# dropbox/lepton

Hardware: AMD Instinct MI355X
Metric: encode+decode MB/s (JPEG bytes/sec), bit-exact round trip (higher is better)
Workload: dtype int16/u8 (integer coder, no floating point)

## Files before the change

### lepton_amd/csrc/lep_dec4.h

```cpp
#pragma once
#include "lep_v3.h"
#include "lep_enc3.h"

namespace lep4 {
using namespace lep3;

#if LEP_ON_GPU && defined(LEP_MARKS)
#define LEP_MARK(name) __asm__ volatile("; MARK " name)
#elif LEP_ON_GPU && defined(LEP_PROF)
#define LEP_MARK(name) prof_stamp(lep4::prof_slot(name))
#else
#define LEP_MARK(name) ((void)0)
#endif
#if LEP_ON_GPU && (defined(LEP_DEC4_PAD_VALU) || defined(LEP_DEC4_PAD_SALU) || defined(LEP_DEC4_PAD_LDS))
#define LEP_PAD8(x) x x x x x x x x
WDEV void pad_block(uint32_t seed, const void* lds) {
    (void)seed; (void)lds;
#ifdef LEP_DEC4_PAD_VALU
    { uint32_t o; for (int i = 0; i < LEP_DEC4_PAD_VALU / 8; ++i) __asm__ volatile(LEP_PAD8("v_add_u32 %0, %1, %1\n") : "=v"(o) : "v"(seed)); }
#endif
#ifdef LEP_DEC4_PAD_SALU
    { uint32_t o; const uint32_t u = uni(seed); for (int i = 0; i < LEP_DEC4_PAD_SALU / 8; ++i) __asm__ volatile(LEP_PAD8("s_add_u32 %0, %1, %1\n") : "=s"(o) : "s"(u) : "scc"); }
#endif
#ifdef LEP_DEC4_PAD_LDS
    { uint32_t o; const uint32_t a = (uint32_t)(uintptr_t)lds; for (int i = 0; i < LEP_DEC4_PAD_LDS / 8; ++i) __asm__ volatile(LEP_PAD8("ds_read_b32 %0, %1\n") "s_waitcnt lgkmcnt(0)\n" : "=v"(o) : "v"(a)); }
#endif
}
#else
WDEV void pad_block(uint32_t, const void*) {}
#endif
constexpr int prof_slot(const char* n) {
    const char* names[18] = {"staging", "prologue", "nz_prefetch", "nz_serial", "nz_update", "77_prefetch", "77_serial", "77_update", "lakhani",
                             "edge_prefetch", "edge_serial", "edge_update", "idct_dcpred", "dc_prefetch", "dc_serial", "dc_update", "publish", "store"};
    for (int i = 0; i < 18; ++i) {
        int k = 0;
        while (names[i][k] && names[i][k] == n[k]) ++k;
        if (!names[i][k] && !n[k]) return i;
    }
    return 31;
}

#ifndef LEP_DEC4_ROW_MAJOR
constexpr uint32_t kGS = 10 * 4;
WDEV uint32_t ctx4_exp7(int ci, int nb, int zz, int bsr) { return lep3::kExp7 + (((((uint32_t)ci * 49 + zz) * 12 + bsr) * 3) * 10 + nb) * 4; }
WDEV uint32_t ctx4_expx(int ci, int ne, int zig15, int bsr) { return lep3::kExpX + (((((uint32_t)ci * 15 + zig15) * 12 + bsr) * 3) * 10 + ne) * 4; }
WDEV uint32_t ctx4_res(int ci, int coord, int nb) { return lep3::kRes + ((((uint32_t)ci * 64 + coord) * 3) * 10 + nb) * 4; }
#else
constexpr uint32_t kGS = 4;
WDEV uint32_t ctx4_exp7(int ci, int nb, int zz, int bsr) { return lep3::ctx_exp7(ci, nb, zz, bsr); }
WDEV uint32_t ctx4_expx(int ci, int ne, int zig15, int bsr) { return lep3::ctx_expx(ci, ne, zig15, bsr); }
WDEV uint32_t ctx4_res(int ci, int coord, int nb) { return lep3::ctx_res(ci, coord, nb); }
#endif
WDEV uint32_t row_word(uint32_t base, int i) { return base + (uint32_t)(i >> 2) * kGS + (uint32_t)(i & 3); }

struct Dec4Shared {
    uint32_t sign[kSignWords];
    uint32_t resdc[kResDcWords];
    alignas(16) int32_t t[64];
    int32_t icos_x[64], icos_y[64];
    int32_t eprior[16];
    int16_t here[64], left[64], above[64], aleft[64];
    alignas(16) int16_t pix[64];
    uint16_t q[64];
    uint8_t thr[64], r2a[64], a2r[64], nzbin[64], bsr[64];
    uint8_t cj[32], cn[32];
    NSum ns_left, ns_above, ns_here;
    uint32_t inv24[512];
};
static_assert(sizeof(Dec4Shared) <= 160 * 1024 / 32, "Dec4Shared no longer fits 32 times into a CU's LDS");

WDEV int nzbin_of(int left) {
    return left < 16 ? (int)((0x7776666555443210ull >> (4 * left)) & 15) : (left < 21 ? 7 : (left < 32 ? 8 : 9));
}
WDEV int nzhi_of(int b) { return (int)((0xc5f50c2050c2040ull >> (6 * b)) & 63); }
#ifndef LEP_DEC4_CANDS
#define LEP_DEC4_CANDS 4
#endif
WDEV int combo_base(int j) { return (int)((0x1b65648d1c0ull >> (6 * j)) & 63); }

WDEV uint32_t inv24_of(uint32_t d) {
    if (d < 2) return 0;
    return (0x1000000u + d - 1) / d - ((d == 337 || d == 469) ? 1u : 0u);
}
WDEV uint32_t mul24(uint32_t a, uint32_t b) {
#if LEP_ON_GPU
    return __umul24(a, b);
#else
    return (uint32_t)(((uint64_t)(a & 0xffffff) * (b & 0xffffff)) & 0xffffffffu);
#endif
}
WDEV uint32_t mul24_low(uint32_t a, uint32_t b) {
#if LEP_ON_GPU
    uint32_t r;
    __asm__("v_mul_u32_u24 %0, %1, %2" : "=v"(r) : "v"(a), "v"(b));
    return r;
#else
    return mul24(a, b);
#endif
}
struct DivBy {
    uint32_t mul, shift;
    WDEV static uint32_t shift_of(uint32_t d) { return 31u - (uint32_t)__builtin_clz(d - 1); }
    WDEV static DivBy of(uint32_t d) {
        DivBy r;
        uint32_t s = 1;
        while (s < 31 && (1u << s) < d) ++s;
        uint32_t q = 0, rem = 1u << (s - 1);
        for (int i = 0; i < 32; ++i) {
            rem <<= 1; q <<= 1;
            if (rem >= d) { rem -= d; q |= 1u; }
        }
        r.mul = q + (rem ? 1u : 0u);
        r.shift = s - 1;
        return r;
    }
};
WDEV uint32_t mulhi_u32(uint32_t a, uint32_t b) {
#if LEP_ON_GPU
    return __umulhi(a, b);
#else
    return (uint32_t)(((uint64_t)a * b) >> 32);
#endif
}
WDEV int32_t div_by(int32_t n, uint32_t mul, uint32_t shift) {
    const int32_t sign = n >> 31;
    const uint32_t u = ((uint32_t)n ^ (uint32_t)sign) - (uint32_t)sign;
    const uint32_t q = mulhi_u32(u, mul) >> shift;
    return (int32_t)((q ^ (uint32_t)sign) - (uint32_t)sign);
}
WDEV uint32_t bupd_t(uint32_t w, uint32_t obs, const uint32_t* inv24) {
    const uint32_t f = (w & 255) + (obs ^ 1), t = ((w >> 8) & 255) + obs;
    uint32_t nw = f | (t << 8) | ((mul24(f << 8, inv24[f + t]) >> 24) << 16);
    if ((f | t) > 255) {
        const uint32_t f0 = w & 255, t0 = (w >> 8) & 255;
        if ((obs ? f0 : t0) == 1) nw = (w & 0xffff) | ((obs ? 0u : 255u) << 16);
        else {
            const uint32_t f2 = obs ? (1 + f0) >> 1 : 129u, t2 = obs ? 129u : (1 + t0) >> 1;
            nw = f2 | (t2 << 8) | ((mul24(f2 << 8, inv24[f2 + t2]) >> 24) << 16);
        }
    }
    return nw;
}
WDEV uint32_t bupd_u(uint32_t w, uint32_t obs, const uint32_t* inv24) {
    const uint32_t w2 = w + 1u + obs * 255u;
    const uint32_t f = w2 & 255u, t = (w2 >> 8) & 255u;
    if (ucond((f < t ? f : t) == 0)) {
        const uint32_t f0 = w & 255, t0 = (w >> 8) & 255;
        if (ucond((obs ? f0 : t0) == 1)) return (w & 0xffff) | ((obs ? 0u : 255u) << 16);
        const uint32_t f2 = obs ? (1 + f0) >> 1 : 129u, t2 = obs ? 129u : (1 + t0) >> 1;
        return f2 | (t2 << 8) | ((mul24(f2 << 8, inv24[f2 + t2]) >> 24) << 16);
    }
    return (w2 & 0xffffu) | (mul24_low(f, inv24[f + t]) & 0xff0000u);
}

WDEV uint64_t pair64(uint32_t hi, uint32_t lo) {
#if LEP_ON_GPU && !defined(LEP_DEC4_PAIR_OR)
    typedef uint32_t u32x2 __attribute__((ext_vector_type(2)));
    const u32x2 p = {lo, hi};
    return __builtin_bit_cast(uint64_t, p);
#else
    return ((uint64_t)hi << 32) | lo;
#endif
}
struct BoolDec4 {
    uint32_t vhi, vlo;
    int count;
    uint32_t range;
    const uint32_t* words;
    uint32_t first, end;
    uint32_t wi;
    uint32_t raw;

    WDEV uint32_t fetch(uint32_t k) const { return k * 4 < end ? words[k] : 0u; }
    WDEV void refill() {
        const uint32_t lo = wi * 4;
        uint32_t w = __builtin_bswap32(raw);
        int nbits = 32;
        if (lo + 4 > end) w = lo < end ? (w & ~(0xffffffffu >> ((end - lo) * 8))) : 0u;
        if (lo < first) { w <<= (first - lo) * 8; nbits -= (int)(first - lo) * 8; }
        const uint64_t add = ((uint64_t)w << 32) >> (count + 8);
        vhi |= (uint32_t)(add >> 32); vlo |= (uint32_t)add;
        count += nbits;
        ++wi;
        raw = fetch(wi);
    }
    WDEV void init_stream(const uint8_t* p, uint32_t n) {
        const uint32_t mis = (uint32_t)((uintptr_t)p & 3);
        words = reinterpret_cast<const uint32_t*>(p - mis);
        first = mis; end = mis + n;
        vhi = vec(0); vlo = vec(0); count = (int)vec((uint32_t)-8); range = vec(255); wi = 0;
        raw = fetch(0);
        refill();
        get(128);
    }
    WDEV uint32_t get(uint32_t prob) {
#if LEP_ON_GPU
        const uint32_t split = 1 + (__umul24(range - 1, prob) >> 8);
#else
        const uint32_t split = 1 + (((range - 1) * prob) >> 8);
#endif
        if (ucond(count < 0)) refill();
        const uint32_t big = split << 24;
        const uint32_t bit = vhi >= big ? 1u : 0u;
        const uint32_t d = vhi - big;
        vhi = d < vhi ? d : vhi;
        range = bit ? range - split : split;
#ifdef LEP_TRACE_GET
        LEP_TRACE_GET(prob, (int)bit);
#endif
        const int shift = __builtin_clz(range) - 24;
        range <<= shift;
        const uint64_t v = pair64(vhi, vlo) << shift;
        vhi = (uint32_t)(v >> 32); vlo = (uint32_t)v;
        count -= shift;
        return bit;
    }
};

struct BoolDec4S {
    uint32_t vhi, vlo;
    int count;
    uint32_t range;
#ifdef LEP_DEC4_RANGE_LOW
    WDEV void load(const BoolDec4& b) { vhi = uni(b.vhi); vlo = uni(b.vlo); count = (int)uni((uint32_t)b.count); range = uni(b.range); }
    WDEV void store(BoolDec4& b) const { b.vhi = vec(vhi); b.vlo = vec(vlo); b.count = (int)vec((uint32_t)count); b.range = vec(range); }
#else
    WDEV void load(const BoolDec4& b) { vhi = uni(b.vhi); vlo = uni(b.vlo); count = (int)uni((uint32_t)b.count); range = uni(b.range) << 24; }
    WDEV void store(BoolDec4& b) const { b.vhi = vec(vhi); b.vlo = vec(vlo); b.count = (int)vec((uint32_t)count); b.range = vec(range >> 24); }
#endif
    WDEV void refill(BoolDec4& b) {
        const uint32_t lo = b.wi * 4;
        uint32_t w = __builtin_bswap32(uni(b.raw));
        int nbits = 32;
        if (lo + 4 > b.end) w = lo < b.end ? (w & ~(0xffffffffu >> ((b.end - lo) * 8))) : 0u;
        if (lo < b.first) { w <<= (b.first - lo) * 8; nbits -= (int)(b.first - lo) * 8; }
        const uint64_t add = ((uint64_t)w << 32) >> (count + 8);
        vhi |= (uint32_t)(add >> 32); vlo |= (uint32_t)add;
        count += nbits;
        ++b.wi;
        b.raw = b.fetch(b.wi);
    }
    WDEV uint32_t get(BoolDec4& b, uint32_t pk) {
        if (count < 0) refill(b);
#ifdef LEP_DEC4_RANGE_LOW
        const uint32_t split = 1 + (((range - 1) * (pk & 255u)) >> 8);
        const uint32_t big = split << 24;
        uint32_t was = vhi;
        const uint32_t bit = was >= big ? 1u : 0u;
        vhi = bit ? was - big : was;
        range = bit ? range - split : split;
        const int shift = __builtin_clz(range) - 24;
#else
        const uint32_t big = ((uint32_t)(((uint64_t)(range - 0x01000000u) * (uint64_t)(pk << 24)) >> 32) & 0xff000000u) + 0x01000000u;
        uint32_t was = vhi;
        const uint32_t bit = was >= big ? 1u : 0u;
        vhi = bit ? was - big : was;
        range = bit ? range - big : big;
        const int shift = __builtin_clz(range);
#endif
#ifdef LEP_TRACE_GET
        LEP_TRACE_GET(pk & 255u, (int)bit);
#endif
        range <<= shift;
        const uint64_t v = pair64(vhi, vlo) << shift;
        vhi = (uint32_t)(v >> 32); vlo = (uint32_t)v;
        count -= shift;
#if LEP_ON_GPU && !defined(LEP_DEC4_PAIR_OR)
        __asm__ volatile("" : "+s"(was));
        return was >= big ? 1u : 0u;
#else
        return bit;
#endif
    }
};

#ifndef LEP_DEC4_PRIO
#define LEP_DEC4_PRIO 1
#endif
#if LEP_ON_GPU && LEP_DEC4_PRIO
#define LEP_PRIO_SERIAL(on_scalar_unit) __builtin_amdgcn_s_setprio((on_scalar_unit) ? 0 : 1)
#define LEP_PRIO_PARALLEL() __builtin_amdgcn_s_setprio(2)
#else
#define LEP_PRIO_SERIAL(on_scalar_unit) ((void)0)
#define LEP_PRIO_PARALLEL() ((void)0)
#endif
#ifndef LEP_DEC4_SCALAR
#define LEP_DEC4_SCALAR 2
#endif

template <int SCMASK>
struct Dec4WaveT {
    const ImageDev* img;
    uint32_t* model;
    Dec4Shared* sh;
    int comp, ci;
    BoolDec4 bc;
    uint32_t nbins;
#if LEP_ON_GPU && !defined(LEP_COUNT_BINS)
#define LEP_BINS(expr) ((void)0)
#else
#define LEP_BINS(expr) (expr)
#endif
#if LEP_ON_GPU && defined(LEP_PROF)
    uint64_t prof_last;
    unsigned long long* prof_out;
    int prof_cur;
    uint32_t prof_acc[20];
    template <int I> __device__ __forceinline__ void prof_add(uint32_t dt) { if (prof_cur == I) prof_acc[I] += dt; }
    __device__ __forceinline__ void prof_stamp(int slot) {
        const uint64_t t = __builtin_readcyclecounter();
        const uint32_t dt = (uint32_t)(t - prof_last);
        prof_last = t;
        prof_add<0>(dt); prof_add<1>(dt); prof_add<2>(dt); prof_add<3>(dt); prof_add<4>(dt); prof_add<5>(dt); prof_add<6>(dt);
        prof_add<7>(dt); prof_add<8>(dt); prof_add<9>(dt); prof_add<10>(dt); prof_add<11>(dt); prof_add<12>(dt); prof_add<13>(dt);
        prof_add<14>(dt); prof_add<15>(dt); prof_add<16>(dt); prof_add<17>(dt); prof_add<18>(dt);
        prof_cur = slot;
    }
    __device__ __forceinline__ void prof_begin(unsigned long long* out) {
        for (int i = 0; i < 20; ++i) prof_acc[i] = 0;
        prof_out = out; prof_cur = 18; prof_last = __builtin_readcyclecounter();
    }
    __device__ __forceinline__ void prof_end() {
        prof_stamp(18);
        if (threadIdx.x == 0) for (int i = 0; i < 19; ++i) prof_out[i] = prof_acc[i];
    }
#endif

    WDEV void init_tables() {
        LANES(l) {
            sh->r2a[l] = kR2A[l]; sh->a2r[l] = kA2R[l]; sh->nzbin[l] = l < 50 ? kNzBin[l] : 9;
            for (int d = l; d < kSignWords; d += 64) sh->sign[d] = kBranchInit;
            for (int d = l; d < kResDcWords; d += 64) sh->resdc[d] = kBranchInit;
            if (l < (int)(sizeof(NSum) / 4)) { ((uint32_t*)&sh->ns_left)[l] = 0; ((uint32_t*)&sh->ns_above)[l] = 0; }
            for (int d = l; d < 512; d += 64) sh->inv24[d] = inv24_of((uint32_t)d);
            if (l < 32) {
                int j = 0, c = l;
                while (j < 6 && c >= 7 - j) { c -= 7 - j; ++j; }
                sh->cj[l] = (uint8_t)(l < 28 ? j : 7); sh->cn[l] = (uint8_t)(l < 28 ? c + 1 : 0);
            }
        }
        LSYNC();
    }
    WDEV void stage_component(int c) {
        comp = c; ci = c ? 1 : 0;
        LANES(l) {
            sh->q[l] = img->q[c][l];
            sh->thr[l] = img->min_thresh[c][l];
            if (l >= 8) { sh->icos_x[l] = img->icos_x[c][l]; sh->icos_y[l] = img->icos_y[c][l]; }
            if (l < 15) {
                const uint32_t d = l < 7 ? (uint32_t)img->icos_x[c][(l + 1) * 8] : (l < 14 ? (uint32_t)img->icos_y[c][(l - 6) * 8] : (uint32_t)img->q[c][0]);
                const DivBy m = DivBy::of(d < 2 || d > 0x7fffffffu ? 2u : d);
                if (l < 7) sh->icos_x[l] = (int32_t)m.mul;
                else if (l < 14) sh->icos_y[l - 7] = (int32_t)m.mul;
                else { sh->icos_x[7] = (int32_t)m.mul; sh->icos_y[7] = d == 1 ? 32 : (int32_t)m.shift; }
            }
        }
        LSYNC();
    }

    template <bool SC>
    struct Serial {
        Dec4WaveT& w;
        BoolDec4S s;
        WDEV explicit Serial(Dec4WaveT& w_) : w(w_) { if (SC) s.load(w.bc); }
        WDEV void done() { if (SC) s.store(w.bc); }
        static WDEV uint32_t U(uint32_t x) { return SC ? uni(x) : vec(x); }
        static WDEV bool is(bool c) { return SC ? c : ucond(c); }
        WDEV uint32_t get(uint32_t prob) { return SC ? s.get(w.bc, prob) : w.bc.get(prob); }
        WDEV uint32_t bupd(uint32_t word, uint32_t obs) {
            if (!SC) return bupd_u(word, obs, w.sh->inv24);
            const uint32_t w2 = word + 1u + obs * 255u;
            const uint32_t f = w2 & 255u, t = (w2 >> 8) & 255u;
            if ((f < t ? f : t) == 0) {
                const uint32_t f0 = word & 255, t0 = (word >> 8) & 255;
                if ((obs ? f0 : t0) == 1) return (word & 0xffff) | ((obs ? 0u : 255u) << 16);
                const uint32_t f2 = obs ? (1 + f0) >> 1 : 129u, t2 = obs ? 129u : (1 + t0) >> 1;
                return f2 | (t2 << 8) | ((((f2 << 8) * uni(w.sh->inv24[f2 + t2])) >> 24) << 16);
            }
            return (w2 & 0xffffu) | ((f * uni(w.sh->inv24[f + t])) & 0xff0000u);
        }
        WDEV uint32_t global_bin(uint32_t idx) {
            const uint32_t word = U(vload(w.model + idx));
            const uint32_t bit = get(word >> 16);
            const uint32_t nw = bupd(word, bit);
#if LEP_ON_GPU
            if (threadIdx.x == 0) w.model[idx] = nw;
#else
            w.model[idx] = nw;
#endif
            return bit;
        }
        template <int K>
        WDEV int unary_from(uint32_t pk) {
            if (K <= 0) { if (!is(get(pk & 255) != 0)) return 0; }
            if (K <= 1) { if (!is(get((pk >> 8) & 255) != 0)) return 1; }
            if (K <= 2) { if (!is(get((pk >> 16) & 255) != 0)) return 2; }
            if (!is(get(pk >> 24) != 0)) return 3;
            return 4;
        }
        WDEV int unary_tail(uint32_t gbase) {
            int i = 8;
#pragma nounroll
            for (; i < 11; ++i) if (!is(global_bin(row_word(gbase, i)) != 0)) break;
            return i;
        }
        WDEV uint32_t residual(uint32_t pk, int b, uint32_t v) {
            if (b >= 3) v |= get(pk >> 24) << 3;
            if (b >= 2) v |= get((pk >> 16) & 255) << 2;
            if (b >= 1) v |= get((pk >> 8) & 255) << 1;
            if (b >= 0) v |= get(pk & 255);
            return v;
        }
        template <int LEVELS>
        WDEV int tree(const uint32_t* PK, int base) {
            uint32_t pk = U(lepwave::wave_read(PK, base));
            uint32_t n = get(pk & 255);
            pk = U(lepwave::wave_read(PK, base + 1));
            n = (n << 1) | get((pk >> (n * 8)) & 255);
            pk = U(lepwave::wave_read(PK, base + 2));
            n = (n << 1) | get((pk >> (n * 8)) & 255);
#pragma unroll
            for (int d = 3; d < LEVELS; ++d) {
                pk = U(lepwave::wave_read(PK, base + (1 << (d - 2)) + 1 + (int)uni(n >> 2)));
                n = (n << 1) | get((pk >> ((n & 3) * 8)) & 255);
            }
            return (int)uni(n);
        }
    };

    static WDEV U4 vload4(const uint32_t* p) {
#if LEP_ON_GPU
        uintptr_t a = (uintptr_t)p;
        __asm__ volatile("" : "+v"(a));
        return ld4(reinterpret_cast<const uint32_t*>(a));
#else
        return ld4(p);
#endif
    }
    static WDEV uint32_t vload(const uint32_t* p) {
#if LEP_ON_GPU
        uintptr_t a = (uintptr_t)p;
        __asm__ volatile("" : "+v"(a));
        return *reinterpret_cast<const uint32_t*>(a);
#else
        return *p;
#endif
    }
    WDEV void idct_rows() { idct_no_dc(sh); }
    static WDEV int half16(int d) { return (int16_t)d / 2; }

    static WDEV void mask_exp(int i0, int len, int& used, int& bits) {
        int n = imin(len, 10) - i0 + 1;
        n = n < 0 ? 0 : (n > 4 ? 4 : n);
        used = (1 << n) - 1;
        const int z = len - i0;
        bits = (z >= 0 && z < 4) ? (used & ~(1 << z)) : used;
    }
    static WDEV void mask_res(int top, int v, int& used, int& bits) {
        top = top > 3 ? 3 : top;
        used = top < 0 ? 0 : (1 << (top + 1)) - 1;
        bits = v & used;
    }
    static WDEV void mask_tree(int i, int k, int value, int& used, int& bits) {
        const int prefix = value >> (i + 1);
        used = (prefix >> 2) == k ? 1 << (prefix & 3) : 0;
        bits = ((value >> i) & 1) ? used : 0;
    }
    template <int ALWAYS>
    WDEV void adapt_group(U4* W, const int* used, const int* bits) {
        const uint32_t* inv = sh->inv24;
#ifdef LEP_DEC4_ADAPT_BRANCHY
        {
            LV(int, any0);
#define LEP_SLOT0(k, fld)                                                                                             \
            LANES(l) L(any0) = (L(used) >> k) & 1;                                                                    \
            if (lepwave::wave_ballot(any0)) {                                                                         \
                LANES(l) if ((L(used) >> k) & 1) L(W).fld = bupd_t(L(W).fld, (uint32_t)(L(bits) >> k) & 1u, inv);    \
            }
            LEP_SLOT0(0, x) LEP_SLOT0(1, y) LEP_SLOT0(2, z) LEP_SLOT0(3, w)
#undef LEP_SLOT0
            return;
        }
#endif
        LV(int, any); LV(uint32_t, oldw); LV(uint32_t, low);
#ifdef LEP_DEC4_ALWAYS_OVERRIDE
        constexpr int kAlways = LEP_DEC4_ALWAYS_OVERRIDE;
#else
        constexpr int kAlways = ALWAYS;
#endif
#define LEP_SLOT(k, fld)                                                                                              \
        if (!((kAlways >> k) & 1)) { LANES(l) L(any) = (L(used) >> k) & 1; }                                           \
        if (((kAlways >> k) & 1) || lepwave::wave_ballot(any)) {                                                       \
            LANES(l) {                                                                                                \
                const uint32_t w = L(W).fld;                                                                          \
                const uint32_t u1 = ((uint32_t)(L(used) & L(bits)) >> k) & 1u, u0 = ((uint32_t)(L(used) & ~L(bits)) >> k) & 1u;   \
                const uint32_t w2 = w + (u0 | (u1 << 8));                                                             \
                const uint32_t f = w2 & 255u, t = (w2 >> 8) & 255u;                                                   \
                const uint32_t p = mul24_low(f, inv[f + t]);    \
                const uint32_t m = mul24(u0 | u1, 0xff0000u);                                                         \
                L(oldw) = w; L(low) = (f < t ? f : t) + ((u0 | u1) ^ 1u);    \
                L(W).fld = (p & m) | (w2 & ~m);                                                                       \
            }                                                                                                         \
            LANES(l) L(any) = L(low) == 0;                                                                            \
            if (lepwave::wave_ballot(any)) {                                                                          \
                LANES(l) if (L(low) == 0) L(W).fld = bupd_t(L(oldw), (uint32_t)(L(bits) >> k) & 1u, inv);             \
            }                                                                                                         \
        }
        LEP_SLOT(0, x) LEP_SLOT(1, y) LEP_SLOT(2, z) LEP_SLOT(3, w)
#undef LEP_SLOT
    }

    WDEV int round_nz(int nzbin_ctx) {
        LEP_MARK("nz_prefetch");
        LV(U4, W0); LV(uint32_t, a0); LV(uint32_t, PK0);
        LANES(l) {
            uint32_t adr = 0, pk = 0;
            if (l < 17) {
                int i, k;
                if (l < 3) { i = 5 - l; k = 0; } else if (l < 5) { i = 2; k = l - 3; } else if (l < 9) { i = 1; k = l - 5; } else { i = 0; k = l - 9; }
                adr = ctx_nz7(ci, nzbin_ctx) + (uint32_t)i * 32 + (uint32_t)k * 4;
                L(W0) = ld4(model + adr); pk = pack_probs(L(W0));
            }
            L(a0) = adr; L(PK0) = pk;
        }
        LEP_MARK("nz_serial"); LEP_PRIO_SERIAL((SCMASK & 1) != 0);
        int nz;
        {
            Serial<(SCMASK & 1) != 0> sr(*this);
            nz = sr.template tree<6>(PK0, 0);
            sr.done();
            LEP_BINS(nbins += 6);
        }
        LEP_MARK("nz_update"); LEP_PRIO_PARALLEL();
        LV(int, u0); LV(int, b0);
        LANES(l) {
            int u = 0, b = 0;
            if (l < 17) {
                int i, k;
                if (l < 3) { i = 5 - l; k = 0; } else if (l < 5) { i = 2; k = l - 3; } else if (l < 9) { i = 1; k = l - 5; } else { i = 0; k = l - 9; }
                mask_tree(i, k, nz, u, b);
            }
            L(u0) = u; L(b0) = b;
        }
        adapt_group<3>(W0, u0, b0);
        LANES(l) if (L(u0)) st4(model + L(a0), L(W0));
        return nz;
    }

    WDEV void round_77(int& zz_io, int& left_io) {
        Dec4Shared& S = *sh;
        LEP_MARK("77_prefetch");
        const int zz0 = zz_io, left0 = left_io, nb0 = nzbin_of(left0);
        LV(U4, W0); LV(U4, W1); LV(uint32_t, a0); LV(uint32_t, a1); LV(uint32_t, PK0); LV(uint32_t, PK1); LV(int, ok);
        LANES(l) {
            const int pi = l & 15, cand = l >> 4, p = zz0 + pi, nb = nb0 - cand;
            uint32_t adr0 = 0, adr1 = 0, pk0 = 0, pk1 = 0;
            const int valid = p < 49 && nb >= 1 && cand < LEP_DEC4_CANDS && pi >= left0 - nzhi_of(nb < 0 ? 0 : nb);
            if (valid) {
                adr0 = ctx4_exp7(ci, nb, p, S.bsr[p]);
                adr1 = ctx4_res(ci, S.a2r[p], nb);
                L(W0) = ld4(model + adr0);
                pk0 = pack_probs(L(W0));
                L(W1) = ld4(model + adr1); pk1 = pack_probs(L(W1));

            }
            L(a0) = adr0; L(a1) = adr1; L(PK0) = pk0; L(PK1) = pk1; L(ok) = valid;
        }
        LSYNC();
        LEP_MARK("77_serial"); LEP_PRIO_SERIAL((SCMASK & 2) != 0);
        int zz, left = left0, cand = 0;
        const int pi_end = zz0 + 16 < 49 ? 16 : 49 - zz0;
        {
            typedef Serial<(SCMASK & 2) != 0> SR;
            SR sr(*this);
            uint32_t sgw = SR::U(S.sign[ci * 48]);
            int pi = 0;
#pragma nounroll
            for (;;) {
                int lane = pi + 16 * cand;
                const int lane_end = pi_end + 16 * cand;
                uint32_t pkv;
                bool found = false;
#pragma nounroll
                for (;;) {
                    pkv = SR::U(lepwave::wave_read(PK0, lane));
                    LEP_BINS(++nbins);
                    if (SR::is(sr.get(pkv & 255) != 0)) { found = true; break; }
                    if (++lane >= lane_end) break;
                }
                pi = lane - 16 * cand;
                if (!found) break;
                zz = zz0 + pi;
                int len = sr.template unary_from<1>(pkv);
                if (len == 4) {
                    len = 4 + sr.template unary_from<0>(SR::U(pack_probs(vload4(model + ctx4_exp7(ci, nb0 - cand, zz, (int)uni(S.bsr[zz])) + kGS))));
                    if (len == 8) len = sr.unary_tail(ctx4_exp7(ci, nb0 - cand, zz, (int)uni(S.bsr[zz])));
                }
                LEP_BINS(nbins += (uint32_t)(2 * len - (len == 11)));
                const uint32_t pos = sr.get(sgw >> 16);
                sgw = sr.bupd(sgw, pos);
                --left;
                uint32_t v = 1u << (len - 1);
                if (len > 1) {
                    int b = len - 2;
                    if (b >= 4) {
                        const uint32_t rbase = ctx4_res(ci, (int)uni(S.a2r[zz]), nb0 - cand);
#pragma nounroll
                        for (; b >= 4; --b) v |= sr.global_bin(row_word(rbase, b)) << b;
                    }
                    v = sr.residual(SR::U(lepwave::wave_read(PK1, lane)), b, v);
                }
                S.here[zz] = (int16_t)(pos ? (int)v : -(int)v);
                ++pi;
                if (left == 0) break;
                cand = nb0 - nzbin_of(left);
                if (cand >= LEP_DEC4_CANDS || pi >= pi_end) break;
            }
            zz = zz0 + pi;
            sr.done();
            S.sign[ci * 48] = sgw;
        }
        LSYNC();
        LEP_MARK("77_update"); LEP_PRIO_PARALLEL();
        LV(int, nzw);
        LANES(l) L(nzw) = l < 16 && zz0 + l < zz && S.here[zz0 + l] != 0;
        const uint32_t nzmask = (uint32_t)lepwave::wave_ballot(nzw);
        LV(int, u0); LV(int, b0); LV(int, u1); LV(int, b1); LV(int, u2); LV(int, b2);
        LANES(l) {
            int ua = 0, ba = 0, ub = 0, bb = 0, uc = 0, bcc = 0;
            const int pi = l & 15, cand_l = l >> 4, p = zz0 + pi;
            if (L(ok) && p < zz) {
                const int left_at = left0 - __builtin_popcount(nzmask & ((1u << pi) - 1));
                if (left_at > 0 && nb0 - (int)S.nzbin[left_at] == cand_l) {
                    const int cf = S.here[p];
                    const int v = cf < 0 ? -cf : cf, len = bitlen((uint32_t)v);
                    mask_exp(0, len, ua, ba);
                    mask_res(len - 2, v, ub, bb);
                    mask_exp(4, len, uc, bcc);
                }
            }
            L(u0) = ua; L(b0) = ba; L(u1) = ub; L(b1) = bb; L(u2) = uc; L(b2) = bcc;
        }
        adapt_group<3>(W0, u0, b0);
        adapt_group<0>(W1, u1, b1);
        LANES(l) {
            if (L(u0)) st4(model + L(a0), L(W0));
            if (L(u1)) st4(model + L(a1), L(W1));
        }
        if (lepwave::wave_ballot(u2)) {
            LV(U4, W2);
            LANES(l) if (L(u2)) L(W2) = ld4(model + L(a0) + kGS);
            adapt_group<0>(W2, u2, b2);
            LANES(l) if (L(u2)) st4(model + L(a0) + kGS, L(W2));
        }
        LSYNC();
        zz_io = zz; left_io = left;
    }

    WDEV int round_edges(int nz, int eob_x, int eob_y, bool has_left, bool has_above) {
        Dec4Shared& S = *sh;
        LEP_MARK("edge_prefetch");
        LV(U4, W0); LV(U4, W1); LV(U4, W2); LV(uint32_t, a0); LV(uint32_t, a2); LV(uint32_t, PK0); LV(uint32_t, PK1); LV(uint32_t, PK2);
        LV(uint32_t, INFO);
        LANES(l) {
            uint32_t adr0 = 0, adr2 = 0, pk0 = 0, pk1 = 0, pk2 = 0, info = 0;
            if (l < 56) {
                const int e = l >= 28 ? 1 : 0, c = l - e * 28, j = S.cj[c], n = S.cn[c];
                const bool horizontal = e == 0;
                const int coord = horizontal ? j + 1 : (j + 1) * 8;
                const int32_t prior = S.eprior[e * 7 + j];
                const uint32_t ap = prior < 0 ? 0u - (uint32_t)prior : (uint32_t)prior;
                const int bsr = bitlen(ap > 1023 ? 1023 : ap);
                adr0 = ctx4_expx(ci, n, horizontal ? j : j + 7, bsr);
                adr2 = ctx4_res(ci, coord, n);
                L(W0) = ld4(model + adr0); L(W2) = ld4(model + adr2);
                pk0 = pack_probs(L(W0)); pk2 = pack_probs(L(W2));
                L(W1) = U4{0, 0, 0, 0};
                const int16_t p16 = (int16_t)prior;
                const int thr = S.thr[coord];
                const uint32_t tctx = (uint32_t)imin((int)((ap & 0xffff) >> thr), 255);
                info = (uint32_t)((ci * 4 + (p16 == 0 ? 0 : (p16 > 0 ? 1 : 2))) * 12 + bsr) | ((uint32_t)thr << 8) | (tctx << 16) |
                       ((uint32_t)bsr << 24) | ((S.eprior[14] >> (e * 7 + j)) & 1 ? 0x80000000u : 0u);
            } else if (l < 62) {
                const int e = l >= 59 ? 1 : 0, lv = l - 56 - 3 * e;
                adr0 = ctx_nzedge(e == 0, ci, e == 0 ? eob_x : eob_y, (nz + 3) / 7) + (uint32_t)(2 - lv) * 4;
                L(W0) = ld4(model + adr0); pk0 = pack_probs(L(W0));
            }
            L(a0) = adr0; L(a2) = adr2; L(PK0) = pk0; L(PK1) = pk1; L(PK2) = pk2; L(INFO) = info;
        }
        LSYNC();
        LEP_MARK("edge_serial"); LEP_PRIO_SERIAL((SCMASK & 4) != 0);
        int ne[2] = {0, 0}, rc = 0;
        typedef Serial<(SCMASK & 4) != 0> SR;
        SR sr(*this);
#pragma nounroll
        for (int e = 0; e < 2 && !rc; ++e) {
            const bool horizontal = e == 0;
            ne[e] = sr.template tree<3>(PK0, 56 + 3 * e);
            LEP_BINS(nbins += 3);
            int left = ne[e];
            if (!left) continue;
            const int a_off = horizontal ? 50 : 57;
            int lane = e * 28 + left - 1, step = 7;
#pragma nounroll
            for (;;) {
                if (SR::is(left > step)) {
#pragma nounroll
                    for (int j = 7 - step; j < 7 && left; ++j) {
                        const uint32_t info = lepwave::wave_read(INFO, e * 28 + combo_base(j));
                        if (info >> 31) { rc = 43; break; }
                        const int coord = horizontal ? j + 1 : (j + 1) * 8;
                        const uint32_t gb = ctx4_expx(ci, left, horizontal ? j : j + 7, (int)((info >> 24) & 15));
                        int len = 0;
#pragma nounroll
                        for (; len < 11; ++len) if (!SR::is(sr.global_bin(row_word(gb, len)) != 0)) break;
                        LEP_BINS(nbins += (uint32_t)(len ? 2 * len + 1 - (len == 11) : 1));
                        if (!len) continue;
                        const int sslot = (int)(info & 255);
                        const uint32_t sgw = SR::U(S.sign[sslot]);
                        const uint32_t pos = sr.get(sgw >> 16);
                        S.sign[sslot] = sr.bupd(sgw, pos);
                        uint32_t v = 1u << (len - 1);
                        int b = len - 2;
                        const int thr = (int)((info >> 8) & 15);
                        if (b >= thr) {
                            const uint32_t Tt = ctx_thresh(ci, (int)((info >> 16) & 255), imin(len - thr, 7));
                            int sx = 1;
#pragma nounroll
                            for (; b >= thr; --b) {
                                const uint32_t bit = sr.global_bin(Tt + (uint32_t)sx);
                                v |= bit << b;
                                sx = imin((sx << 1) | (int)uni(bit), 127);
                            }
                        }
                        const uint32_t rbase = ctx4_res(ci, coord, left);
#pragma nounroll
                        for (; b >= 0; --b) v |= sr.global_bin(row_word(rbase, b)) << b;
                        S.here[a_off + j] = (int16_t)(pos ? (int)v : -(int)v);
                        --left;
                    }
                    break;
                }
                const uint32_t info = lepwave::wave_read(INFO, lane);
                if (info >> 31) { rc = 43; break; }
                const uint32_t pkv = SR::U(lepwave::wave_read(PK0, lane));
                LEP_BINS(++nbins);
                if (SR::is(sr.get(pkv & 255) != 0)) {
                    const int j = 7 - step;
                    const int coord = horizontal ? j + 1 : (j + 1) * 8;
                    int len = sr.template unary_from<1>(pkv);
                    if (len == 4) {
                        len = 4 + sr.template unary_from<0>(SR::U(pack_probs(vload4(model + ctx4_expx(ci, left, horizontal ? j : j + 7, (int)((info >> 24) & 15)) + kGS))));
                        if (len == 8) len = sr.unary_tail(ctx4_expx(ci, left, horizontal ? j : j + 7, (int)((info >> 24) & 15)));
                    }
                    LEP_BINS(nbins += (uint32_t)(2 * len - (len == 11)));
                    const int sslot = (int)(info & 255);
                    const uint32_t sgw = SR::U(S.sign[sslot]);
                    const uint32_t pos = sr.get(sgw >> 16);
                    S.sign[sslot] = sr.bupd(sgw, pos);
                    uint32_t v = 1u << (len - 1);
                    if (len > 1) {
                        int b = len - 2;
                        const int thr = (int)((info >> 8) & 15);
                        if (b >= thr) {
                            const uint32_t Tt = ctx_thresh(ci, (int)((info >> 16) & 255), imin(len - thr, 7));
                            int sx = 1;
#pragma nounroll
                            for (; b >= thr; --b) {
                                const uint32_t bit = sr.global_bin(Tt + (uint32_t)sx);
                                v |= bit << b;
                                sx = imin((sx << 1) | (int)uni(bit), 127);
                            }
                        }
                        if (b >= 4) {
                            const uint32_t rbase = ctx4_res(ci, coord, left);
#pragma nounroll
                            for (; b >= 4; --b) v |= sr.global_bin(row_word(rbase, b)) << b;
                        }
                        v = sr.residual(SR::U(lepwave::wave_read(PK2, lane)), b, v);
                    }
                    S.here[a_off + j] = (int16_t)(pos ? (int)v : -(int)v);
                    --lane;
                    if (--left == 0) break;
                }
                lane += step;
                if (--step == 0) break;
            }
        }
        sr.done();
        LSYNC();
        if (rc) return rc;
        LEP_MARK("edge_update"); LEP_PRIO_PARALLEL();
        LV(int, enz);
        LANES(l) L(enz) = l >= 50 && S.here[l] != 0;
        const uint64_t em = lepwave::wave_ballot(enz);
        const uint32_t mh = (uint32_t)(em >> 50) & 0x7f, mv = (uint32_t)(em >> 57) & 0x7f;
        const int neh = ne[0], nev = ne[1];
        LV(int, u0); LV(int, b0); LV(int, u1); LV(int, b1); LV(int, u2); LV(int, b2);
        LANES(l) {
            int ua = 0, ba = 0, ub = 0, bb = 0, uc = 0, bcc = 0;
            if (l < 56) {
                const int e = l >= 28 ? 1 : 0, c = l - e * 28, j = S.cj[c], n = S.cn[c];
                const uint32_t mk = e ? mv : mh;
                const int left_at = (e ? nev : neh) - __builtin_popcount(mk & ((1u << j) - 1));
                if (left_at == n) {
                    const int cf = S.here[(e ? 57 : 50) + j];
                    const int v = cf < 0 ? -cf : cf, len = bitlen((uint32_t)v);
                    mask_exp(0, len, ua, ba);
                    mask_exp(4, len, ub, bb);
                    mask_res(imin(len - 2, (int)S.thr[e ? (j + 1) * 8 : j + 1] - 1), v, uc, bcc);
                }
            } else if (l < 62) {
                const int e = l >= 59 ? 1 : 0, lv = l - 56 - 3 * e;
                mask_tree(2 - lv, 0, e ? nev : neh, ua, ba);
            }
            L(u0) = ua; L(b0) = ba; L(u1) = ub; L(b1) = bb; L(u2) = uc; L(b2) = bcc;
        }
        adapt_group<3>(W0, u0, b0);
        LANES(l) if (L(u0)) st4(model + L(a0), L(W0));
        if (lepwave::wave_ballot(u1)) {
            LANES(l) if (L(u1)) L(W1) = ld4(model + L(a0) + kGS);
            adapt_group<0>(W1, u1, b1);
            LANES(l) if (L(u1)) st4(model + L(a0) + kGS, L(W1));
        }
        if (lepwave::wave_ballot(u2)) {
            adapt_group<0>(W2, u2, b2);
            LANES(l) if (L(u2)) st4(model + L(a2), L(W2));
        }
        LSYNC();
        return 0;
    }

    WDEV void round_dc(int pred, int a, int b17, int sctx) {
        Dec4Shared& S = *sh;
        LEP_MARK("dc_prefetch");
        LV(U4, W0); LV(uint32_t, a0); LV(uint32_t, PK0); LV(uint32_t, RW);
        LANES(l) {
            uint32_t adr = 0, pk = 0, rw = 0;
            if (l < 3) { adr = ctx_expdc(a, b17) + (uint32_t)l * 4; L(W0) = ld4(model + adr); pk = pack_probs(L(W0)); }
            else if (l < 13) rw = S.resdc[a * 12 + (l - 3)];
            L(a0) = adr; L(PK0) = pk; L(RW) = rw;
        }
        LEP_MARK("dc_serial"); LEP_PRIO_SERIAL((SCMASK & 8) != 0);
        const int sslot = ci * 48 + sctx;
        typedef Serial<(SCMASK & 8) != 0> SR;
        SR sr(*this);
        int len = sr.template unary_from<0>(SR::U(lepwave::wave_read(PK0, 0)));
        if (len == 4) {
            len += sr.template unary_from<0>(SR::U(lepwave::wave_read(PK0, 1)));
            if (len == 8) {
                uint32_t pk = SR::U(lepwave::wave_read(PK0, 2));
#pragma nounroll
                for (; len < 11; ++len) { if (!SR::is(sr.get(pk & 255) != 0)) break; pk >>= 8; }
            }
        }
        LEP_BINS(nbins += (uint32_t)(len ? 2 * len + 1 - (len == 11) : 1));
        uint32_t v = 0, pos = 1;
        if (len) {
            const uint32_t sgw = SR::U(S.sign[sslot]);
            pos = sr.get(sgw >> 16);
            S.sign[sslot] = sr.bupd(sgw, pos);
            v = 1u << (len - 1);
#pragma nounroll
            for (int i = len - 2; i >= 0; --i) v |= sr.get(SR::U(lepwave::wave_read(RW, 3 + i)) >> 16) << i;
        }
        sr.done();
        v = vec(v);
        int d = (int16_t)(pos ? (int)v : -(int)v);
        int dc = d + pred;
        dc = dc < -1024 ? dc + 2049 : dc;
        dc = dc > 1024 ? dc - 2049 : dc;
        S.here[49] = (int16_t)dc;
        LSYNC();
        LEP_MARK("dc_update"); LEP_PRIO_PARALLEL();
        LV(uint32_t, VV); LV(int, u0); LV(int, b0);
        LANES(l) L(VV) = v;
        LANES(l) {
            int u = 0, b = 0;
            if (l < 3) mask_exp(l * 4, len, u, b);
            L(u0) = u; L(b0) = b;
        }
        adapt_group<7>(W0, u0, b0);
        LANES(l) {
            if (L(u0)) st4(model + L(a0), L(W0));
            if (l >= 3 && l < 13 && l - 3 <= len - 2) S.resdc[a * 12 + (l - 3)] = bupd_t(L(RW), (L(VV) >> (l - 3)) & 1u, S.inv24);
        }
        LSYNC();
    }

    WDEV int decode_block(bool has_left, bool has_above) {
        Dec4Shared& S = *sh;
        LEP_MARK("prologue");
        LANES(l) {
            S.here[l] = 0;
            if (l < 49) {
                int prior;
                if (has_left && has_above) prior = (uint16_t)((iabs(S.left[l]) + iabs(S.above[l])) * 13 + 6 * iabs(S.aleft[l])) >> 5;
                else if (has_left) prior = (int16_t)iabs(S.left[l]);
                else if (has_above) prior = (int16_t)iabs(S.above[l]);
                else prior = 0;
                S.bsr[l] = (uint8_t)bitlen((uint32_t)imin(iabs(prior), 1023));
            }
        }
        int nzctx = 0;
        if (has_left && has_above) nzctx = (S.ns_above.nz + S.ns_left.nz + 2) / 4;
        else if (has_above) nzctx = (S.ns_above.nz + 1) / 2;
        else if (has_left) nzctx = (S.ns_left.nz + 1) / 2;
        const int nzbin_ctx = (int)uni((uint32_t)nzbin_of(nzctx));
        LSYNC();

        const int nz = round_nz(nzbin_ctx);
        if (nz > 49) return 7;
        {
            int zz = 0, left = nz;
#pragma nounroll
            while (zz < 49 && left > 0) round_77(zz, left);
        }
        LEP_MARK("lakhani");
        int eob_x, eob_y;
        {
            LV(int, tx); LV(int, ty); LV(int, badf);
            LANES(l) {
                int ex = 0, ey = 0, bad = 0;
                if (l < 49 && S.here[l] != 0) { const int coord = S.a2r[l]; ex = coord & 7; ey = coord >> 3; }
                if (l < 14) {
                    const bool hz = l < 7;
                    const int j = hz ? l : l - 7;
                    const int coord = hz ? j + 1 : (j + 1) * 8;
                    int32_t prior = 0;
                    if (hz ? has_above : has_left) {
                        const int16_t* nbr = hz ? S.above : S.left;
                        const int32_t* icos = hz ? S.icos_x + coord * 8 : S.icos_y + coord;
                        const int step = hz ? 8 : 1;
                        if (icos[0] != 0) {
                            uint32_t acc = (uint32_t)(int32_t)nbr[S.r2a[coord]] * (uint32_t)icos[0];
                            for (int i = 1; i < 8; ++i) {
                                int32_t xi = S.here[S.r2a[coord + i * step]], ai = nbr[S.r2a[coord + i * step]];
                                int32_t term = (i & 1) ? xi + ai : xi - ai;
                                acc -= (uint32_t)icos[i] * (uint32_t)term;
                            }
                            prior = div_by((int32_t)acc, (uint32_t)(hz ? S.icos_x[j] : S.icos_y[j]), DivBy::shift_of((uint32_t)icos[0]));
                        } else bad = 1;
                    }
                    S.eprior[l] = prior;
                }
                L(tx) = ex; L(ty) = ey; L(badf) = bad;
            }
            eob_x = lepwave::wave_max(tx); eob_y = lepwave::wave_max(ty);
            const uint64_t badmask = lepwave::wave_ballot(badf);
            LANES(l) if (l == 0) S.eprior[14] = (int32_t)(uint32_t)badmask;
            LSYNC();
        }
        {
            const int rc = round_edges(nz, eob_x, eob_y, has_left, has_above);
            if (rc) return rc;
        }
        LEP_MARK("idct_dcpred");
        idct_rows();
        int pred, a, b17, sctx;
        {
            LV(int, emin); LV(int, emax); LV(int, s0); LV(int, s1); LV(int, tmp);
            LANES(l) {
                int ev = 0, have = 0;
                if (l < 8 && has_left) { have = 1; ev = (int16_t)(S.ns_left.vert[l] - half16(LEP_PIX(S, l, 0) - LEP_PIX(S, l, 1)) - (LEP_PIX(S, l, 0) + 1024)); }
                if (l >= 8 && l < 16 && has_above) { const int i = l - 8; have = 1; ev = (int16_t)(S.ns_above.horiz[i] - half16(LEP_PIX(S, 0, i) - LEP_PIX(S, 1, i)) - (LEP_PIX(S, 0, i) + 1024)); }
                L(emax) = have ? ev : -0x7fffffff;
                L(emin) = have ? -ev : -0x7fffffff;
                L(s0) = l < 8 ? ev : 0;
                L(s1) = (l >= 8 && l < 16) ? ev : 0;
            }
            const int mx = lepwave::wave_max(emax), mn = -lepwave::wave_max(emin);
            const int sumL = lepwave::wave_sum(s0), sumA = lepwave::wave_sum(s1);
            int32_t avgmed = 0, unc = 0, unc2 = 0;
            if (has_left || has_above) {
                int sum0 = has_left ? sumL : sumA, sum1 = (has_left && has_above) ? sumA : sum0;
                avgmed = (sum0 + sum1) >> 1;
                unc = (mx - mn) >> 3;
                sum0 -= avgmed; sum1 -= avgmed;
                unc2 = (iabs(sum0) < iabs(sum1) ? sum0 : sum1) >> 3;
            }
            const uint32_t dc_shift = (uint32_t)S.icos_y[7];
            pred = ((dc_shift == 32 ? avgmed : div_by(avgmed, (uint32_t)S.icos_x[7], dc_shift)) + 4) >> 3;
            a = imin(bitlen((uint32_t)iabs(unc) & 0xffff), 11);
            b17 = imin(bitlen((uint32_t)iabs(unc2) & 0xffff), 16);
            sctx = unc2 >= 0 ? (unc2 == 0 ? 3 : 2) : 1;
        }
        round_dc(pred, a, b17, sctx);
        LEP_MARK("publish");
        pad_block((uint32_t)pred, sh);
        LANES(l) {
            if (l < 16) {
                const int i = l & 7;
                const int dcq = S.here[49] * (int)S.q[0];
                if (l < 8) S.ns_here.horiz[i] = (int16_t)(dcq + LEP_PIX(S, 7, i) + 1024 + half16(LEP_PIX(S, 7, i) - LEP_PIX(S, 6, i)));
                else S.ns_here.vert[i] = (int16_t)(dcq + LEP_PIX(S, i, 7) + 1024 + half16(LEP_PIX(S, i, 7) - LEP_PIX(S, i, 6)));
            }
            if (l == 16) S.ns_here.nz = nz;
        }
        LSYNC();
        return 0;
    }

    WDEV int run(const ImageDev* image, const SegDev& seg, uint32_t* model_words, NSum* ns, Dec4Shared* shared, const uint8_t* stream,
                 uint32_t len) {
        img = image; model = model_words; sh = shared; nbins = 0;
        LEP_PRIO_PARALLEL();
        init_tables();
        bc.init_stream(stream, len);
        bool top[3] = {true, true, true};
        for (uint32_t idx = 0;; ++idx) {
            RowSpec r = row_spec(image, idx);
            if (r.done) break;
            if (r.luma_y >= seg.y1 && !seg.is_last) break;
            if (r.skip) continue;
            if (r.luma_y < seg.y0) continue;
            stage_component(r.component);
            const int w = img->width[comp], yb = r.curr_y;
            int16_t* row = img->blocks[comp] + (int64_t)yb * w * 64;
            const bool has_above = !top[comp];
            const int16_t* arow = has_above ? row - (int64_t)w * 64 : nullptr;
            NSum* nrow = ns + img->ns_offset[comp] + (yb & 1) * w;
            const NSum* narow = ns + img->ns_offset[comp] + ((yb & 1) ^ 1) * w;
            top[comp] = false;
            LV(int16_t, nxt_above); LV(uint32_t, nxt_ns);
            LANES(l) {
                L(nxt_above) = has_above ? arow[l] : (int16_t)0;
                L(nxt_ns) = (has_above && l < (int)(sizeof(NSum) / 4)) ? ((const uint32_t*)&narow[0])[l] : 0u;
            }
            const int coded_here = (int)img->coded_blocks[comp] - yb * w;
            const int x_end = imin(w, coded_here < 1 ? 1 : coded_here);
            for (int x = 0; x < x_end; ++x) {
                LEP_MARK("staging");
        LANES(l) {
                    if (x) { sh->left[l] = sh->here[l]; sh->aleft[l] = sh->above[l]; }
                    if (l < (int)(sizeof(NSum) / 4)) {
                        if (x) ((uint32_t*)&sh->ns_left)[l] = ((const uint32_t*)&sh->ns_here)[l];
                        if (has_above) ((uint32_t*)&sh->ns_above)[l] = L(nxt_ns);
                    }
                }
                LSYNC();
                LANES(l) {
                    if (has_above) sh->above[l] = L(nxt_above);
                    if (has_above && x + 1 < x_end) {
                        L(nxt_above) = arow[(int64_t)(x + 1) * 64 + l];
                        if (l < (int)(sizeof(NSum) / 4)) L(nxt_ns) = ((const uint32_t*)&narow[x + 1])[l];
                    }
                }
                LSYNC();
                int rc = decode_block(x > 0, has_above);
                if (rc) return rc;
                LEP_MARK("store");
        LANES(l) {
                    row[(int64_t)x * 64 + l] = sh->here[l];
                    if (l < (int)(sizeof(NSum) / 4)) ((uint32_t*)&nrow[x])[l] = ((const uint32_t*)&sh->ns_here)[l];
                }
            }
        }
        return 0;
    }
};
typedef Dec4WaveT<LEP_DEC4_SCALAR> Dec4Wave;

}
```

Baseline: 1576.

## Batch bool-decoder refills and streamline branch-free model adaptation in dec4

Adds an ensure(n) refill check so unary, residual and tree decode loops can call a no-check get, removing the per-bin refill branch. The group adaptation in adapt_group becomes a branch-free update with a rare redo path for saturated counters. A per-lane single-word adapt_word is added for the nz and dc update stages, replacing the 4-wide group adapt with one word per lane. All three are enabled by default through the LEP_DEC4_DIET=7 bitmask. The risk is a bit-exactness mismatch if the redo path or the ensure bit budget is wrong.

```diff
diff --git a/lepton_amd/csrc/lep_dec4.h b/lepton_amd/csrc/lep_dec4.h
--- a/lepton_amd/csrc/lep_dec4.h
+++ b/lepton_amd/csrc/lep_dec4.h
@@ -76,6 +76,16 @@
 #ifndef LEP_DEC4_CANDS
 #define LEP_DEC4_CANDS 4
 #endif
+#ifndef LEP_DEC4_DIET
+#define LEP_DEC4_DIET 7
+#endif
+#if !LEP_ON_GPU && defined(LEP_COUNT_REDO)
+static uint32_t redo_count[4];
+extern "C" __attribute__((used, visibility("default"))) uint32_t* lep_dec4_redo_count() { return redo_count; }
+#define LEP_REDO_SEEN(i) (++lep4::redo_count[i])
+#else
+#define LEP_REDO_SEEN(i) ((void)0)
+#endif
 WDEV int combo_base(int j) { return (int)((0x1b65648d1c0ull >> (6 * j)) & 63); }
 
 WDEV uint32_t inv24_of(uint32_t d) {
@@ -140,6 +150,9 @@
         }
     }
     return nw;
+}
+WDEV uint32_t bupd_redo(uint32_t wn, uint32_t obs, const uint32_t* inv24) {
+    return bupd_t(obs ? ((wn & 0xffu) | 0xff00u) : (0xffu | ((((wn >> 8) - 1u) & 0xffu) << 8)), obs, inv24);
 }
 WDEV uint32_t bupd_u(uint32_t w, uint32_t obs, const uint32_t* inv24) {
     const uint32_t w2 = w + 1u + obs * 255u;
@@ -193,13 +206,17 @@
         refill();
         get(128);
     }
+    WDEV void ensure(int n) { if (ucond(count < 7 * (n - 1))) refill(); }
     WDEV uint32_t get(uint32_t prob) {
+        if (ucond(count < 0)) refill();
+        return get_nocheck(prob);
+    }
+    WDEV uint32_t get_nocheck(uint32_t prob) {
 #if LEP_ON_GPU
         const uint32_t split = 1 + (__umul24(range - 1, prob) >> 8);
 #else
         const uint32_t split = 1 + (((range - 1) * prob) >> 8);
 #endif
-        if (ucond(count < 0)) refill();
         const uint32_t big = split << 24;
         const uint32_t bit = vhi >= big ? 1u : 0u;
         const uint32_t d = vhi - big;
@@ -367,6 +384,13 @@
         static WDEV uint32_t U(uint32_t x) { return SC ? uni(x) : vec(x); }
         static WDEV bool is(bool c) { return SC ? c : ucond(c); }
         WDEV uint32_t get(uint32_t prob) { return SC ? s.get(w.bc, prob) : w.bc.get(prob); }
+#if LEP_DEC4_DIET & 4
+        WDEV void ensure(int n) { if (!SC) w.bc.ensure(n); }
+        WDEV uint32_t getn(uint32_t prob) { return SC ? s.get(w.bc, prob) : w.bc.get_nocheck(prob); }
+#else
+        WDEV void ensure(int) {}
+        WDEV uint32_t getn(uint32_t prob) { return get(prob); }
+#endif
         WDEV uint32_t bupd(uint32_t word, uint32_t obs) {
             if (!SC) return bupd_u(word, obs, w.sh->inv24);
             const uint32_t w2 = word + 1u + obs * 255u;
@@ -392,10 +416,11 @@
         }
         template <int K>
         WDEV int unary_from(uint32_t pk) {
-            if (K <= 0) { if (!is(get(pk & 255) != 0)) return 0; }
-            if (K <= 1) { if (!is(get((pk >> 8) & 255) != 0)) return 1; }
-            if (K <= 2) { if (!is(get((pk >> 16) & 255) != 0)) return 2; }
-            if (!is(get(pk >> 24) != 0)) return 3;
+            ensure(K <= 0 ? 4 : 4 - K);
+            if (K <= 0) { if (!is(getn(pk & 255) != 0)) return 0; }
+            if (K <= 1) { if (!is(getn((pk >> 8) & 255) != 0)) return 1; }
+            if (K <= 2) { if (!is(getn((pk >> 16) & 255) != 0)) return 2; }
+            if (!is(getn(pk >> 24) != 0)) return 3;
             return 4;
         }
         WDEV int unary_tail(uint32_t gbase) {
@@ -405,24 +430,27 @@
             return i;
         }
         WDEV uint32_t residual(uint32_t pk, int b, uint32_t v) {
-            if (b >= 3) v |= get(pk >> 24) << 3;
-            if (b >= 2) v |= get((pk >> 16) & 255) << 2;
-            if (b >= 1) v |= get((pk >> 8) & 255) << 1;
-            if (b >= 0) v |= get(pk & 255);
+            ensure(4);
+            if (b >= 3) v |= getn(pk >> 24) << 3;
+            if (b >= 2) v |= getn((pk >> 16) & 255) << 2;
+            if (b >= 1) v |= getn((pk >> 8) & 255) << 1;
+            if (b >= 0) v |= getn(pk & 255);
             return v;
         }
         template <int LEVELS>
         WDEV int tree(const uint32_t* PK, int base) {
+            ensure(3);
             uint32_t pk = U(lepwave::wave_read(PK, base));
-            uint32_t n = get(pk & 255);
+            uint32_t n = getn(pk & 255);
             pk = U(lepwave::wave_read(PK, base + 1));
-            n = (n << 1) | get((pk >> (n * 8)) & 255);
+            n = (n << 1) | getn((pk >> (n * 8)) & 255);
             pk = U(lepwave::wave_read(PK, base + 2));
-            n = (n << 1) | get((pk >> (n * 8)) & 255);
+            n = (n << 1) | getn((pk >> (n * 8)) & 255);
+            if (LEVELS > 3) ensure(LEVELS - 3 > 4 ? 4 : LEVELS - 3);
 #pragma unroll
             for (int d = 3; d < LEVELS; ++d) {
                 pk = U(lepwave::wave_read(PK, base + (1 << (d - 2)) + 1 + (int)uni(n >> 2)));
-                n = (n << 1) | get((pk >> ((n & 3) * 8)) & 255);
+                n = (n << 1) | getn((pk >> ((n & 3) * 8)) & 255);
             }
             return (int)uni(n);
         }
@@ -482,12 +510,46 @@
             return;
         }
 #endif
-        LV(int, any); LV(uint32_t, oldw); LV(uint32_t, low);
 #ifdef LEP_DEC4_ALWAYS_OVERRIDE
         constexpr int kAlways = LEP_DEC4_ALWAYS_OVERRIDE;
 #else
         constexpr int kAlways = ALWAYS;
 #endif
+#if LEP_DEC4_DIET & 2
+        LV(int, any); LV(uint32_t, low);
+        LANES(l) L(low) = 255u;
+        do {
+#define LEP_SLOT(k, fld)                                                                                              \
+            if (!((kAlways >> k) & 1)) {                                                                               \
+                LANES(l) L(any) = (uint32_t)L(used) > (1u << k) - 1u;                                                  \
+                if (!lepwave::wave_ballot(any)) break;                                                                \
+            }                                                                                                         \
+            LANES(l) {                                                                                                \
+                const uint32_t w = L(W).fld;                                                                          \
+                const uint32_t u1 = ((uint32_t)(L(used) & L(bits)) >> k) & 1u, u0 = ((uint32_t)(L(used) & ~L(bits)) >> k) & 1u;   \
+                const uint32_t w2 = w + (u0 | (u1 << 8));                                                             \
+                const uint32_t f = w2 & 255u, t = (w2 >> 8) & 255u;                                                   \
+                const uint32_t p = mul24_low(f, inv[f + t]);    \
+                const uint32_t m = mul24(u0 | u1, 0xff0000u);                                                         \
+                const uint32_t lo = L(low) < f ? L(low) : f;                                                          \
+                L(low) = lo < t ? lo : t;                                                                             \
+                L(W).fld = (p & m) | (w2 & ~m);                                                                       \
+            }
+            LEP_SLOT(0, x) LEP_SLOT(1, y) LEP_SLOT(2, z) LEP_SLOT(3, w)
+#undef LEP_SLOT
+        } while (0);
+        LANES(l) L(any) = L(low) == 0 && L(used) != 0;
+        if (lepwave::wave_ballot(any)) {
+#define LEP_REDO(k, fld)                                                                                              \
+            LANES(l) if (L(any) && ((L(used) >> k) & 1)) {                                                            \
+                const uint32_t obs = (uint32_t)(L(bits) >> k) & 1u, wn = L(W).fld;                                    \
+                if (((obs ? wn >> 8 : wn) & 255u) == 0) { L(W).fld = bupd_redo(wn, obs, inv); LEP_REDO_SEEN(0); }     \
+            }
+            LEP_REDO(0, x) LEP_REDO(1, y) LEP_REDO(2, z) LEP_REDO(3, w)
+#undef LEP_REDO
+        }
+#else
+        LV(int, any); LV(uint32_t, oldw); LV(uint32_t, low);
 #define LEP_SLOT(k, fld)                                                                                              \
         if (!((kAlways >> k) & 1)) { LANES(l) L(any) = (L(used) >> k) & 1; }                                           \
         if (((kAlways >> k) & 1) || lepwave::wave_ballot(any)) {                                                       \
@@ -508,6 +570,24 @@
         }
         LEP_SLOT(0, x) LEP_SLOT(1, y) LEP_SLOT(2, z) LEP_SLOT(3, w)
 #undef LEP_SLOT
+#endif
+    }
+    WDEV void adapt_word(uint32_t* Wd, const int* on, const int* obs, int site_lo, int site_hi) {
+        (void)site_lo; (void)site_hi;
+        const uint32_t* inv = sh->inv24;
+        LV(int, any);
+        LANES(l) {
+            const uint32_t u = (uint32_t)L(on), o = (uint32_t)L(obs);
+            const uint32_t w2 = L(Wd) + (u << (o << 3));
+            const uint32_t f = w2 & 255u, t = (w2 >> 8) & 255u;
+            const uint32_t p = mul24_low(f, inv[f + t]);
+            const uint32_t m = mul24(u, 0xff0000u);
+            L(any) = (int)u & (int)((f < t ? f : t) == 0);
+            L(Wd) = (p & m) | (w2 & ~m);
+        }
+        if (lepwave::wave_ballot(any)) {
+            LANES(l) if (L(any)) { L(Wd) = bupd_redo(L(Wd), (uint32_t)L(obs), inv); LEP_REDO_SEEN(l < 16 ? site_lo : site_hi); }
+        }
     }
 
     WDEV int round_nz(int nzbin_ctx) {
@@ -533,6 +613,24 @@
         }
         LEP_MARK("nz_update"); LEP_PRIO_PARALLEL();
         LV(int, u0); LV(int, b0);
+#if LEP_DEC4_DIET & 1
+        LV(uint32_t, WD);
+        LANES(l) {
+            int u = 0, b = 0;
+            uint32_t wd = 0;
+            if (l < 17) {
+                int i, k;
+                if (l < 3) { i = 5 - l; k = 0; } else if (l < 5) { i = 2; k = l - 3; } else if (l < 9) { i = 1; k = l - 5; } else { i = 0; k = l - 9; }
+                const int prefix = nz >> (i + 1), sl = prefix & 3;
+                u = (prefix >> 2) == k; b = (nz >> i) & 1;
+                wd = sl == 0 ? L(W0).x : (sl == 1 ? L(W0).y : (sl == 2 ? L(W0).z : L(W0).w));
+                L(a0) += (uint32_t)sl;
+            }
+            L(u0) = u; L(b0) = b; L(WD) = wd;
+        }
+        adapt_word(WD, u0, b0, 1, 1);
+        LANES(l) if (L(u0)) model[L(a0)] = L(WD);
+#else
         LANES(l) {
             int u = 0, b = 0;
             if (l < 17) {
@@ -544,6 +642,7 @@
         }
         adapt_group<3>(W0, u0, b0);
         LANES(l) if (L(u0)) st4(model + L(a0), L(W0));
+#endif
         return nz;
     }
 
@@ -839,6 +938,9 @@
             uint32_t adr = 0, pk = 0, rw = 0;
             if (l < 3) { adr = ctx_expdc(a, b17) + (uint32_t)l * 4; L(W0) = ld4(model + adr); pk = pack_probs(L(W0)); }
             else if (l < 13) rw = S.resdc[a * 12 + (l - 3)];
+#if LEP_DEC4_DIET & 1
+            else if (l >= 16 && l < 27) { adr = ctx_expdc(a, b17) + (uint32_t)(l - 16); rw = model[adr]; }
+#endif
             L(a0) = adr; L(PK0) = pk; L(RW) = rw;
         }
         LEP_MARK("dc_serial"); LEP_PRIO_SERIAL((SCMASK & 8) != 0);
@@ -875,6 +977,19 @@
         LEP_MARK("dc_update"); LEP_PRIO_PARALLEL();
         LV(uint32_t, VV); LV(int, u0); LV(int, b0);
         LANES(l) L(VV) = v;
+#if LEP_DEC4_DIET & 1
+        LANES(l) {
+            int u = 0, b = 0;
+            if (l >= 3 && l < 13) { u = l - 3 <= len - 2; b = (int)((L(VV) >> (l - 3)) & 1u); }
+            else if (l >= 16 && l < 27) { u = l - 16 <= imin(len, 10); b = l - 16 != len; }
+            L(u0) = u; L(b0) = b;
+        }
+        adapt_word(RW, u0, b0, 2, 3);
+        LANES(l) if (L(u0)) {
+            if (l < 16) S.resdc[a * 12 + (l - 3)] = L(RW);
+            else model[L(a0)] = L(RW);
+        }
+#else
         LANES(l) {
             int u = 0, b = 0;
             if (l < 3) mask_exp(l * 4, len, u, b);
@@ -885,6 +1000,7 @@
             if (L(u0)) st4(model + L(a0), L(W0));
             if (l >= 3 && l < 13 && l - 3 <= len - 2) S.resdc[a * 12 + (l - 3)] = bupd_t(L(RW), (L(VV) >> (l - 3)) & 1u, S.inv24);
         }
+#endif
         LSYNC();
     }
 
```

Result: no change. 1592 (median of 6 runs) (+1.0%).
